# Aazmp/vp8oclenc

Measured on AMD Instinct MI355X. Metric: macroblocks/sec inter-frame (ME+DCT+loopfilter), 1080p, higher is better.
Workload: dtype u8/int32

## Files before the change

vp8oclenc_amd/csrc/kernels_s2.hip:

```cpp
#include <stdlib.h>
#include <string.h>

#include "vp8hip_dev.h"
#include "kernels_rc_dev.h"

namespace vp8 {

namespace {

constexpr uint32_t pk8(int a, int b, int c, int d) {
    return (uint32_t)(a & 255) | ((uint32_t)(b & 255) << 8) | ((uint32_t)(c & 255) << 16) | ((uint32_t)(d & 255) << 24);
}
constexpr int TAPS[5][6] = {{3, -16, 77, 77, -16, 3}, {1, -8, 36, 108, -11, 2}, {0, 0, 128, 0, 0, 0}, {2, -11, 108, 36, -8, 1}, {3, -16, 77, 77, -16, 3}};
struct OperandTable { uint32_t w[64][4]; };
constexpr OperandTable make_bh() {
    OperandTable t{};
    for (int l = 0; l < 64; ++l) {
        const int n = l & 31, xi = n >> 3, c = n & 7, xc = xi + (xi >> 1), s = xc >= 2 ? 1 : 0;
        for (int j = 0; j < 16; ++j) {
            const int k = 16 * (l >> 5) + j, tap = k - c - s;
            const int v = k == 31 ? 64 : (tap >= 0 && tap < 6) ? TAPS[xc][tap] : 0;
            t.w[l][j >> 2] |= (uint32_t)(v & 255) << (8 * (j & 3));
        }
    }
    return t;
}
constexpr OperandTable make_av() {
    OperandTable t{};
    for (int l = 0; l < 64; ++l) {
        const int m = l & 31, f = m >> 3, i = m & 7, yc = f + (f >> 1), s = yc >= 2 ? 1 : 0;
        for (int j = 0; j < 16; ++j) {
            const int k = 16 * (l >> 5) + j, tap = k - i - s;
            const int v = k == 31 ? 64 : (tap >= 0 && tap < 6) ? TAPS[yc][tap] : 0;
            t.w[l][j >> 2] |= (uint32_t)(v & 255) << (8 * (j & 3));
        }
    }
    return t;
}
static __device__ __constant__ const OperandTable K_BH = make_bh();
static __device__ __constant__ const OperandTable K_AV = make_av();

constexpr int HT_XC = 36;
constexpr int V_STRIDE = 20;
constexpr int WIN_ROW = 8;
__device__ __forceinline__ void lds_fence() { asm volatile("s_waitcnt lgkmcnt(0)" ::: "memory"); }

struct S2Args {
    Plane cur;
    Plane ref[3];
    const int16_t *net_in[3];
    int16_t *net_out[3];
    int32_t *bdiff[3];
    int refmap[3];
    int nrefs;
    int w, h, nblk, bw;
    uint32_t bw_inv;
    unsigned long long *clk;
};

__device__ __forceinline__ uint32_t umin(uint32_t a, uint32_t b) { return a < b ? a : b; }
template <int CTRL, int ROW_MASK = 0xf>
__device__ __forceinline__ uint32_t dpp(uint32_t v) {
    return (uint32_t)__builtin_amdgcn_update_dpp((int)v, (int)v, CTRL, ROW_MASK, 0xf, false);
}
template <int CTRL, int ROW_MASK = 0xf>
__device__ __forceinline__ uint32_t dpp_or_max(uint32_t v) {
    return (uint32_t)__builtin_amdgcn_update_dpp(-1, (int)v, CTRL, ROW_MASK, 0xf, false);
}
__device__ __forceinline__ uint32_t halfwave_min_upper(uint32_t key) {
    key = umin(key, dpp_or_max<0xb1>(key));
    key = umin(key, dpp_or_max<0x4e>(key));
    key = umin(key, dpp_or_max<0x141>(key));
    key = umin(key, dpp_or_max<0x140>(key));
    return umin(key, dpp_or_max<0x142, 0xa>(key));
}

typedef unsigned short us2 __attribute__((ext_vector_type(2)));
__device__ __forceinline__ unsigned short ashr7_pk_i8(int a, int b) { return __builtin_amdgcn_ashr_pk_i8_i32(a, b, 7); }
__device__ __forceinline__ uint32_t pack4(unsigned short lo, unsigned short hi) {
    const us2 v = {lo, hi};
    return __builtin_bit_cast(uint32_t, v);
}
__device__ __forceinline__ uint32_t round_pack4(const v16i &acc, int q) {
    return pack4(ashr7_pk_i8(acc[4 * q], acc[4 * q + 1]), ashr7_pk_i8(acc[4 * q + 2], acc[4 * q + 3]));
}
__device__ __forceinline__ v4i one_at_k31(v4i d, int upper) {
    d.w = (int)(((uint32_t)d.w & (0xffffffffu >> (8 & upper))) | (0x01000000u & (uint32_t)upper));
    return d;
}
__device__ __forceinline__ v16i mfma_round(v4i a, v4i b) {
    const v16i c = {0, 0, 0, 0, 0, 0, 0, 0, 0, 0, 0, 0, 0, 0, 0, 0};
    return __builtin_amdgcn_mfma_i32_32x32x32_i8(a, b, c, 0, 0, 0);
}

template <bool SPREAD>
__device__ __forceinline__ void search2_body(const S2Args &a, int wg_x, int ref_idx, int tn) {
    if (ref_idx >= a.nrefs) return;
    __shared__ __attribute__((aligned(16))) uint32_t s_HT[8][5 * HT_XC];
    __shared__ __attribute__((aligned(16))) uint32_t s_cz[8][32];
    __shared__ __attribute__((aligned(16))) uint32_t s_V[8][25 * V_STRIDE];
    uint32_t(*s_win)[25 * V_STRIDE] = s_V;
    int(*s_pre)[5 * HT_XC] = reinterpret_cast<int(*)[5 * HT_XC]>(s_HT);
    const int r = a.refmap[ref_idx];
    const int g = threadIdx.x >> 5, lane = threadIdx.x & 31;
    const int b = imin(wg_x * 8 + g, a.nblk - 1);
    const bool live = wg_x * 8 + g < a.nblk;
    const int by = a.bw == 1 ? b : (int)__umulhi((uint32_t)b, a.bw_inv), bx = b - by * a.bw;
    const int cx = bx * 8, cy = by * 8;
    const uint32_t nv = reinterpret_cast<const uint32_t *>(a.net_in[r])[b];
    const int nx = (int16_t)(nv & 0xffffu), ny = (int16_t)(nv >> 16);
    const int v0x = (int16_t)(nx * 4), v0y = (int16_t)(ny * 4);
    const int Lx = iclamp(cx + nx, 3 - EXT, a.w + EXT - 11), Ly = iclamp(cy + ny, 3 - EXT, a.h + EXT - 11);
    const Plane rf = a.ref[r];
    const int wl = threadIdx.x & 63, kh = wl >> 5, gp = g & ~1;
    const int g_n = tn >> 5, lane_n = tn & 31, wl_n = tn & 63, kh_n = wl_n >> 5, gp_n = g_n & ~1;
    {
        const int row = lane_n >> 1, half = lane_n & 1;
        v4i v;
        __builtin_memcpy(&v, rf.p + (ptrdiff_t)(Ly - 3 + row) * rf.stride + (Lx - 3) + 16 * half, 16);
        *reinterpret_cast<v4i *>(&s_win[g_n][row * WIN_ROW + 4 * half]) = v ^ (int)0x80808080u;
    }
    {
        const int sel = lane_n >> 4, row = (lane_n >> 1) & 7, half = lane_n & 1;
        const uint8_t *base = sel ? rf.p : a.cur.p;
        const int stride = sel ? rf.stride : a.cur.stride;
        const uint32_t v = *reinterpret_cast<const uint32_t *>(base + (ptrdiff_t)(cy + row) * stride + cx + 4 * half) ^ 0x80808080u;
        uint8_t *cz = reinterpret_cast<uint8_t *>(s_cz[g_n]) + sel * 64 + half * 32 + row;
#pragma unroll
        for (int j = 0; j < 4; ++j) cz[j * 8] = (uint8_t)(v >> (8 * j));
    }
    lds_fence();

    {
        const int m = wl & 31, m_n = wl_n & 31;
        const v4i aw = *reinterpret_cast<const v4i *>(&s_win[gp_n + (m_n >> 4)][(m_n & 15) * WIN_ROW + 4 * kh_n]);
        const v4i bh = *reinterpret_cast<const v4i *>(K_BH.w[wl_n]);
        const v16i acc = mfma_round(one_at_k31(aw, -kh_n), bh);
        const int xi = m >> 3, c = m & 7, xc = xi + (xi >> 1);
        uint32_t *ht = &s_HT[gp][xc * HT_XC + c * 4 + kh];
#pragma unroll
        for (int q = 0; q < 4; ++q) ht[(q >> 1) * (5 * HT_XC) + 2 * (q & 1)] = round_pack4(acc, q);
    }
    {
        const int c = lane_n & 7, rg = lane_n >> 3;
        const uint8_t *wb = reinterpret_cast<const uint8_t *>(s_win[g_n]) + 3 + c + rg * (16 * WIN_ROW);
        uint32_t v = 0;
#pragma unroll
        for (int rr = 0; rr < 4; ++rr) v |= (uint32_t)wb[rr * (4 * WIN_ROW)] << (8 * rr);
        s_HT[g_n][2 * HT_XC + c * 4 + rg] = v;
    }
    lds_fence();

    {
        const v4i av = *reinterpret_cast<const v4i *>(K_AV.w[wl_n]);
#pragma unroll
        for (int t = 0; t < 3; ++t) {
            const int ng = 32 * t + (wl & 31);
            const bool on = t < 2 || (wl & 31) < 16;
            const int blk = ng >= 40 ? 1 : 0, rem = on ? ng - 40 * blk : 0, xc = rem >> 3, c = rem & 7;
            const v4i hv = *reinterpret_cast<const v4i *>(&s_HT[gp + blk][xc * HT_XC + c * 4]);
            const v16i acc = mfma_round(av, one_at_k31(hv, -kh_n));
            if (on) {
                uint32_t *sv = &s_V[gp + blk][xc * V_STRIDE + c * 2 + kh];
#pragma unroll
                for (int f = 0; f < 4; ++f) sv[(f + (f >> 1)) * 5 * V_STRIDE] = round_pack4(acc, f);
                sv[2 * 5 * V_STRIDE] = kh ? __builtin_amdgcn_alignbyte((uint32_t)hv[2], (uint32_t)hv[1], 3)
                                          : __builtin_amdgcn_alignbyte((uint32_t)hv[1], (uint32_t)hv[0], 3);
            }
        }
    }
    lds_fence();
    {
        const int q = lane_n & 15, m = q >> 3, n = (q >> 2) & 1, j = q & 3;
        const uint32_t ccol = s_cz[g_n][(4 * n + j) * 2 + m];
        int *pre = &s_pre[g_n][q * 4 + (lane_n >> 4) * 2];
        pre[0] = dot4s(ccol, lane_n < 16 ? K_W_R0 : K_W_X, 0);
        pre[1] = dot4s(ccol, lane_n < 16 ? K_W_R2 : K_W_Y, 0);
    }
    lds_fence();

    const int k = lane;
    const int dx = k % 5 - 2, dy = k / 5 - 2;
    int qx = (int16_t)(cx * 4 + v0x + dx), qy = (int16_t)(cy * 4 + v0y + dy);
    if (k == 25) { qx = cx * 4; qy = cy * 4; }
    const bool valid = live && k < 26 && qx >= 0 && qx <= a.w * 4 - 32 && qy >= 0 && qy <= a.h * 4 - 32;
    int diff = 0;
    const v4i wa = metric_a(wl_n);
    auto cols4 = [](const uint32_t *src) { return v4i{(int)src[0], (int)src[2], (int)src[4], (int)src[6]}; };
    if (SPREAD) {
        int *q3 = &s_pre[g][64];
        const bool helper = lane >= 26;
        const uint32_t *own = k < 25 ? &s_V[g][k * V_STRIDE] : &s_cz[g][16];
        const uint32_t *hsrc = &s_V[g][(lane - 26) * 3 * V_STRIDE + 9];
        int *hdst = &q3[(lane - 26) * 3];
        auto metric = [&](const uint32_t *src, const int *pre16) { return weight_mfma(wa, load_pre16(pre16), cols4(src)); };
#pragma unroll
        for (int j = 0; j < 3; ++j) {
            const int c = metric(helper ? hsrc + j * V_STRIDE : own + (8 * (j & 1) + (j >> 1)), &s_pre[g][helper ? 48 : 16 * j]);
            *(helper ? hdst + j : &q3[31]) = c;
            diff += helper ? 0 : c;
        }
        __syncthreads();
        if ((int)(threadIdx.x >> 6) == (wg_x & 3)) {
            const int slot = wl >> 3, cand = 18 + (wl & 7);
            s_pre[slot][64 + cand] = metric((cand < 25 ? &s_V[slot][cand * V_STRIDE] : &s_cz[slot][16]) + 9, &s_pre[slot][48]);
        }
        __syncthreads();
        diff += q3[k < 26 ? k : 31];
    } else {
    const uint32_t *src = k < 25 ? &s_V[g][k * V_STRIDE] : &s_cz[g][16];
#pragma unroll
    for (int m = 0; m < 2; ++m)
#pragma unroll
        for (int n = 0; n < 2; ++n) diff += weight_mfma(wa, load_pre16(&s_pre[g][(m * 2 + n) * 16]), cols4(src + 8 * n + m));
    }
    if (k < 25) diff += (iabs(dx) + iabs(dy)) * 32;
    uint32_t key = (valid && diff < 0x7fff) ? ((uint32_t)diff << 8) | (uint32_t)k : 0xffffffffu;
    key = halfwave_min_upper(key);
    if (lane == 16 && live) {
        int bqx = (int16_t)(a.w * 4 - 32), bqy = (int16_t)(a.h * 4 - 32), md = 0x7fff;
        if (key != 0xffffffffu) {
            const int kk = key & 0xff;
            md = (int)(key >> 8);
            bqx = kk == 25 ? cx * 4 : (int16_t)(cx * 4 + v0x + (kk % 5 - 2));
            bqy = kk == 25 ? cy * 4 : (int16_t)(cy * 4 + v0y + (kk / 5 - 2));
        }
        const int vx = (int16_t)(bqx - cx * 4), vy = (int16_t)(bqy - cy * 4);
        if ((vx != 0) | (vy != 0)) md -= (iabs(vx - v0x) + iabs(vy - v0y)) * 32;
        reinterpret_cast<uint32_t *>(a.net_out[r])[b] = (uint32_t)(uint16_t)vx | ((uint32_t)(uint16_t)vy << 16);
        a.bdiff[r][b] = md;
    }
}

template <bool SPREAD, int ITER>
__device__ __forceinline__ void search2_groups(const S2Args &a, int grp, int ref_idx) {
    if (ITER == 1) { search2_body<SPREAD>(a, grp, ref_idx, (int)threadIdx.x); return; }
#pragma unroll 1
    for (int it = 0; it < ITER; ++it) {
        int tn = (int)threadIdx.x;
        asm volatile("" : "+v"(tn));
        search2_body<SPREAD>(a, grp * ITER + it, ref_idx, tn);
    }
}
template <bool SPREAD, int ITER>
__global__ __launch_bounds__(256, 4) void k_search2(S2Args a) {
    launch_clock_begin(a.clk);
    search2_groups<SPREAD, ITER>(a, xcd_band(blockIdx.x, gridDim.x), blockIdx.y);
    launch_clock_end(a.clk);
}
static_assert(sizeof(BatchOf<S2Args>) <= 4096, "a batch's argument blocks travel in the 4 KiB kernel-argument segment");
template <bool SPREAD, int ITER>
__global__ __launch_bounds__(256, 4) void k_search2_b(BatchOf<S2Args> b) {
    launch_clock_begin(b.item[0].clk);
    search2_groups<SPREAD, ITER>(b.item[blockIdx.z], xcd_band(blockIdx.x, gridDim.x), blockIdx.y);
    launch_clock_end(b.item[0].clk);
}
struct S2Scans { rc::ScanCore item[MAX_BATCH]; uint32_t mask; int nbx, wgs; };
static_assert(sizeof(BatchOf<S2Args>) + sizeof(S2Scans) <= 4096, "the kernel-argument segment");
template <bool SPREAD, int ITER>
__global__ __attribute__((amdgpu_waves_per_eu(7, 8))) __launch_bounds__(256) void k_search2_bs(BatchOf<S2Args> b, S2Scans sc) {
    if ((int)blockIdx.x >= sc.nbx) {
        const int wg = (int)blockIdx.x - sc.nbx;
        if (blockIdx.y == 0 && ((sc.mask >> blockIdx.z) & 1) && wg < sc.wgs) rc::strength_segments_body(b.item[blockIdx.z].cur, sc.item[blockIdx.z], wg, sc.wgs);
        return;
    }
    launch_clock_begin(b.item[0].clk);
    search2_groups<SPREAD, ITER>(b.item[blockIdx.z], xcd_band(blockIdx.x, sc.nbx), blockIdx.y);
    launch_clock_end(b.item[0].clk);
}
__global__ __launch_bounds__(256, 4) void k_search2_p(BatchOf<S2Args> b, int nbx, int maxrefs, int total) {
    for (int w = blockIdx.x; w < total; w += gridDim.x) {
        const int item = w / (nbx * maxrefs), rem = w - item * (nbx * maxrefs);
        const int ref_idx = rem / nbx, wg_x = rem - ref_idx * nbx;
        search2_body<false>(b.item[item], wg_x, ref_idx, (int)threadIdx.x);
        lds_fence();
    }
}

}

static S2Args search2_args(const Frame &cur, const RefSet &refs, const NetSet &nets, unsigned long long *clk) {
    S2Args a;
    a.clk = clk;
    a.cur = cur.Y[0];
    int n = 0;
    for (int r = 0; r < 3; ++r) {
        a.ref[r] = refs.ref[r].Y[0];
        a.net_in[r] = nets.net[r][1];
        a.net_out[r] = nets.net[r][0];
        a.bdiff[r] = nets.bdiff[r];
        if (refs.use[r]) a.refmap[n++] = r;
    }
    a.nrefs = n;
    for (int i = n; i < 3; ++i) a.refmap[i] = 0;
    a.w = a.cur.w;
    a.h = a.cur.h;
    a.bw = a.w / 8;
    a.bw_inv = (uint32_t)(((1ull << 32) + a.bw - 1) / a.bw);
    a.nblk = a.w * a.h / 64;
    return a;
}
static bool search2_spread() {
    static const bool on = [] { const char *v = getenv("VP8HIP_S2_SPREAD"); return !(v && v[0] == '0'); }();
    return on;
}
static int search2_iter(bool batch) {
    static const int forced = [] { const char *v = getenv("VP8HIP_S2_ITER"); const int k = v && v[0] ? atoi(v) : 0; return k == 1 || k == 2 || k == 4 ? k : 0; }();
    return forced ? forced : (batch ? 4 : 1);
}
static bool search2_skip() {
    static const bool skip = experiment_skip("s2");
    return skip;
}

void launch_search2(hipStream_t s, const Frame &cur, const RefSet &refs, const NetSet &nets, unsigned long long *clk) {
    const S2Args a = search2_args(cur, refs, nets, clk);
    if (a.nrefs == 0 || search2_skip()) return;
    const int nbx = (a.nblk + 7) / 8;
    if (!search2_spread()) VP8_LAUNCH((k_search2<false, 1>), dim3(nbx, a.nrefs), dim3(256), 0, s, a);
    else if (search2_iter(false) == 4) VP8_LAUNCH((k_search2<true, 4>), dim3((nbx + 3) / 4, a.nrefs), dim3(256), 0, s, a);
    else if (search2_iter(false) == 2) VP8_LAUNCH((k_search2<true, 2>), dim3((nbx + 1) / 2, a.nrefs), dim3(256), 0, s, a);
    else VP8_LAUNCH((k_search2<true, 1>), dim3(nbx, a.nrefs), dim3(256), 0, s, a);
}

bool launch_search2_batch(hipStream_t s, const Frame *const *cur, const RefSet *refs, const NetSet *const *nets, int n, unsigned long long *clk,
                          const ScanRequest *const *scan) {
    BatchOf<S2Args> b;
    b.n = n;
    int maxrefs = 0;
    for (int i = 0; i < n; ++i) {
        b.item[i] = search2_args(*cur[i], refs[i], *nets[i], clk);
        maxrefs = b.item[i].nrefs > maxrefs ? b.item[i].nrefs : maxrefs;
    }
    if (maxrefs == 0 || search2_skip()) return false;
    const int nbx = (b.item[0].nblk + 7) / 8;
    const int persist = persistent_workgroups();
    if (persist > 0 && nbx * maxrefs * n > persist) {
        VP8_LAUNCH(k_search2_p, dim3(persist), dim3(256), 0, s, b, nbx, maxrefs, nbx * maxrefs * n);
        return false;
    }
    S2Scans sc;
    sc.mask = 0;
    for (int i = 0; scan && i < n; ++i) {
        if (!scan[i]) continue;
        const ScanRequest &q = *scan[i];
        const Plane &y = b.item[i].cur;
        sc.mask |= 1u << i;
        sc.item[i] = rc::ScanCore{q.partial, q.partial + 2 * rc::MAX_PARTIALS, q.stats, q.sd, q.strength_out,
                                  rc::SegArgs{y.w * y.h, (y.h - 1) * (y.w - 1), q.is_key, q.refqi[0], q.refqi[1], q.refqi[2], q.refqi[3], q.qi_min}};
    }
    const int iter = search2_spread() ? search2_iter(true) : 1, ngrp = (nbx + iter - 1) / iter;
    if (!sc.mask) {
        if (!search2_spread()) VP8_LAUNCH((k_search2_b<false, 1>), dim3(nbx, maxrefs, n), dim3(256), 0, s, b);
        else if (iter == 4) VP8_LAUNCH((k_search2_b<true, 4>), dim3(ngrp, maxrefs, n), dim3(256), 0, s, b);
        else if (iter == 2) VP8_LAUNCH((k_search2_b<true, 2>), dim3(ngrp, maxrefs, n), dim3(256), 0, s, b);
        else VP8_LAUNCH((k_search2_b<true, 1>), dim3(nbx, maxrefs, n), dim3(256), 0, s, b);
        return false;
    }
    sc.nbx = ngrp;
    sc.wgs = (b.item[0].h + rc::ROWS_PER_BLOCK - 1) / rc::ROWS_PER_BLOCK;
    if (!search2_spread()) VP8_LAUNCH((k_search2_bs<false, 1>), dim3(nbx + sc.wgs, maxrefs, n), dim3(256), 0, s, b, sc);
    else if (iter == 4) VP8_LAUNCH((k_search2_bs<true, 4>), dim3(ngrp + sc.wgs, maxrefs, n), dim3(256), 0, s, b, sc);
    else if (iter == 2) VP8_LAUNCH((k_search2_bs<true, 2>), dim3(ngrp + sc.wgs, maxrefs, n), dim3(256), 0, s, b, sc);
    else VP8_LAUNCH((k_search2_bs<true, 1>), dim3(nbx + sc.wgs, maxrefs, n), dim3(256), 0, s, b, sc);
    return true;
}

}
```

Baseline: 69.19 million.

## Loop over all references inside one search2 workgroup and relayout subpel buffer

Batched search2 kernels now process every reference frame inside a single workgroup instead of one grid row per reference. The current-block precompute (dot products against the metric weights) is done once and reused across references. The interpolated-candidate LDS buffer is relaid so each candidate's four columns are contiguous and can be read with one vector load. The zero-MV reference block is stored into the same buffer. Default ITER for batches drops from 4 to 2 and the non-batch kernel switches to a waves_per_eu occupancy hint. This trades fewer workgroups and less parallelism for less redundant current-block work and fewer launches, with larger LDS per group.

```diff
diff --git a/vp8oclenc_amd/csrc/kernels_s2.hip b/vp8oclenc_amd/csrc/kernels_s2.hip
--- a/vp8oclenc_amd/csrc/kernels_s2.hip
+++ b/vp8oclenc_amd/csrc/kernels_s2.hip
@@ -41,7 +41,11 @@
 static __device__ __constant__ const OperandTable K_AV = make_av();
 
 constexpr int HT_XC = 36;
-constexpr int V_STRIDE = 20;
+constexpr int V_CAND = 4;
+constexpr int V_ROW = 26 * V_CAND;
+constexpr int V_SLOT = 4 * V_ROW;
+constexpr int V_ZERO = 25;
+constexpr int PRE_SLOT = 96;
 constexpr int WIN_ROW = 8;
 __device__ __forceinline__ void lds_fence() { asm volatile("s_waitcnt lgkmcnt(0)" ::: "memory"); }
 
@@ -93,166 +97,184 @@
     return __builtin_amdgcn_mfma_i32_32x32x32_i8(a, b, c, 0, 0, 0);
 }
 
-template <bool SPREAD>
+template <bool SPREAD, bool ALLREFS>
 __device__ __forceinline__ void search2_body(const S2Args &a, int wg_x, int ref_idx, int tn) {
-    if (ref_idx >= a.nrefs) return;
+    if (ALLREFS ? a.nrefs == 0 : ref_idx >= a.nrefs) return;
     __shared__ __attribute__((aligned(16))) uint32_t s_HT[8][5 * HT_XC];
-    __shared__ __attribute__((aligned(16))) uint32_t s_cz[8][32];
-    __shared__ __attribute__((aligned(16))) uint32_t s_V[8][25 * V_STRIDE];
-    uint32_t(*s_win)[25 * V_STRIDE] = s_V;
-    int(*s_pre)[5 * HT_XC] = reinterpret_cast<int(*)[5 * HT_XC]>(s_HT);
-    const int r = a.refmap[ref_idx];
+    __shared__ __attribute__((aligned(16))) uint32_t s_V[8][V_SLOT];
+    uint32_t(*s_win)[V_SLOT] = s_V;
+    __shared__ __attribute__((aligned(16))) int s_pre[8][PRE_SLOT];
+    int(*s_q3)[5 * HT_XC] = reinterpret_cast<int(*)[5 * HT_XC]>(s_HT);
     const int g = threadIdx.x >> 5, lane = threadIdx.x & 31;
+    const int wl = threadIdx.x & 63, kh = wl >> 5, gp = g & ~1;
     const int b = imin(wg_x * 8 + g, a.nblk - 1);
     const bool live = wg_x * 8 + g < a.nblk;
     const int by = a.bw == 1 ? b : (int)__umulhi((uint32_t)b, a.bw_inv), bx = b - by * a.bw;
     const int cx = bx * 8, cy = by * 8;
-    const uint32_t nv = reinterpret_cast<const uint32_t *>(a.net_in[r])[b];
-    const int nx = (int16_t)(nv & 0xffffu), ny = (int16_t)(nv >> 16);
-    const int v0x = (int16_t)(nx * 4), v0y = (int16_t)(ny * 4);
-    const int Lx = iclamp(cx + nx, 3 - EXT, a.w + EXT - 11), Ly = iclamp(cy + ny, 3 - EXT, a.h + EXT - 11);
-    const Plane rf = a.ref[r];
-    const int wl = threadIdx.x & 63, kh = wl >> 5, gp = g & ~1;
-    const int g_n = tn >> 5, lane_n = tn & 31, wl_n = tn & 63, kh_n = wl_n >> 5, gp_n = g_n & ~1;
     {
-        const int row = lane_n >> 1, half = lane_n & 1;
-        v4i v;
-        __builtin_memcpy(&v, rf.p + (ptrdiff_t)(Ly - 3 + row) * rf.stride + (Lx - 3) + 16 * half, 16);
-        *reinterpret_cast<v4i *>(&s_win[g_n][row * WIN_ROW + 4 * half]) = v ^ (int)0x80808080u;
-    }
-    {
-        const int sel = lane_n >> 4, row = (lane_n >> 1) & 7, half = lane_n & 1;
-        const uint8_t *base = sel ? rf.p : a.cur.p;
-        const int stride = sel ? rf.stride : a.cur.stride;
-        const uint32_t v = *reinterpret_cast<const uint32_t *>(base + (ptrdiff_t)(cy + row) * stride + cx + 4 * half) ^ 0x80808080u;
-        uint8_t *cz = reinterpret_cast<uint8_t *>(s_cz[g_n]) + sel * 64 + half * 32 + row;
-#pragma unroll
-        for (int j = 0; j < 4; ++j) cz[j * 8] = (uint8_t)(v >> (8 * j));
-    }
-    lds_fence();
-
-    {
-        const int m = wl & 31, m_n = wl_n & 31;
-        const v4i aw = *reinterpret_cast<const v4i *>(&s_win[gp_n + (m_n >> 4)][(m_n & 15) * WIN_ROW + 4 * kh_n]);
-        const v4i bh = *reinterpret_cast<const v4i *>(K_BH.w[wl_n]);
-        const v16i acc = mfma_round(one_at_k31(aw, -kh_n), bh);
-        const int xi = m >> 3, c = m & 7, xc = xi + (xi >> 1);
-        uint32_t *ht = &s_HT[gp][xc * HT_XC + c * 4 + kh];
-#pragma unroll
-        for (int q = 0; q < 4; ++q) ht[(q >> 1) * (5 * HT_XC) + 2 * (q & 1)] = round_pack4(acc, q);
-    }
-    {
-        const int c = lane_n & 7, rg = lane_n >> 3;
-        const uint8_t *wb = reinterpret_cast<const uint8_t *>(s_win[g_n]) + 3 + c + rg * (16 * WIN_ROW);
-        uint32_t v = 0;
-#pragma unroll
-        for (int rr = 0; rr < 4; ++rr) v |= (uint32_t)wb[rr * (4 * WIN_ROW)] << (8 * rr);
-        s_HT[g_n][2 * HT_XC + c * 4 + rg] = v;
-    }
-    lds_fence();
-
-    {
-        const v4i av = *reinterpret_cast<const v4i *>(K_AV.w[wl_n]);
-#pragma unroll
-        for (int t = 0; t < 3; ++t) {
-            const int ng = 32 * t + (wl & 31);
-            const bool on = t < 2 || (wl & 31) < 16;
-            const int blk = ng >= 40 ? 1 : 0, rem = on ? ng - 40 * blk : 0, xc = rem >> 3, c = rem & 7;
-            const v4i hv = *reinterpret_cast<const v4i *>(&s_HT[gp + blk][xc * HT_XC + c * 4]);
-            const v16i acc = mfma_round(av, one_at_k31(hv, -kh_n));
-            if (on) {
-                uint32_t *sv = &s_V[gp + blk][xc * V_STRIDE + c * 2 + kh];
-#pragma unroll
-                for (int f = 0; f < 4; ++f) sv[(f + (f >> 1)) * 5 * V_STRIDE] = round_pack4(acc, f);
-                sv[2 * 5 * V_STRIDE] = kh ? __builtin_amdgcn_alignbyte((uint32_t)hv[2], (uint32_t)hv[1], 3)
-                                          : __builtin_amdgcn_alignbyte((uint32_t)hv[1], (uint32_t)hv[0], 3);
-            }
-        }
-    }
-    lds_fence();
-    {
+        const int g_n = tn >> 5, lane_n = tn & 31;
+        uint32_t *tmp = reinterpret_cast<uint32_t *>(&s_pre[g_n][80]);
+        if (lane_n < 16) {
+            const int row = lane_n >> 1, half = lane_n & 1;
+            const uint32_t v = *reinterpret_cast<const uint32_t *>(a.cur.p + (ptrdiff_t)(cy + row) * a.cur.stride + cx + 4 * half) ^ 0x80808080u;
+            uint8_t *cz = reinterpret_cast<uint8_t *>(tmp) + half * 32 + row;
+#pragma unroll
+            for (int j = 0; j < 4; ++j) cz[j * 8] = (uint8_t)(v >> (8 * j));
+        }
+        lds_fence();
         const int q = lane_n & 15, m = q >> 3, n = (q >> 2) & 1, j = q & 3;
-        const uint32_t ccol = s_cz[g_n][(4 * n + j) * 2 + m];
+        const uint32_t ccol = tmp[(4 * n + j) * 2 + m];
         int *pre = &s_pre[g_n][q * 4 + (lane_n >> 4) * 2];
-        pre[0] = dot4s(ccol, lane_n < 16 ? K_W_R0 : K_W_X, 0);
-        pre[1] = dot4s(ccol, lane_n < 16 ? K_W_R2 : K_W_Y, 0);
-    }
-    lds_fence();
-
+        const int p0 = dot4s(ccol, lane_n < 16 ? K_W_R0 : K_W_X, 0), p1 = dot4s(ccol, lane_n < 16 ? K_W_R2 : K_W_Y, 0);
+        pre[0] = p0;
+        pre[1] = p1;
+        if (q >= 12) { pre[16] = p0; pre[17] = p1; pre[32] = p0; pre[33] = p1; }
+    }
     const int k = lane;
     const int dx = k % 5 - 2, dy = k / 5 - 2;
-    int qx = (int16_t)(cx * 4 + v0x + dx), qy = (int16_t)(cy * 4 + v0y + dy);
-    if (k == 25) { qx = cx * 4; qy = cy * 4; }
-    const bool valid = live && k < 26 && qx >= 0 && qx <= a.w * 4 - 32 && qy >= 0 && qy <= a.h * 4 - 32;
-    int diff = 0;
-    const v4i wa = metric_a(wl_n);
-    auto cols4 = [](const uint32_t *src) { return v4i{(int)src[0], (int)src[2], (int)src[4], (int)src[6]}; };
-    if (SPREAD) {
-        int *q3 = &s_pre[g][64];
-        const bool helper = lane >= 26;
-        const uint32_t *own = k < 25 ? &s_V[g][k * V_STRIDE] : &s_cz[g][16];
-        const uint32_t *hsrc = &s_V[g][(lane - 26) * 3 * V_STRIDE + 9];
-        int *hdst = &q3[(lane - 26) * 3];
-        auto metric = [&](const uint32_t *src, const int *pre16) { return weight_mfma(wa, load_pre16(pre16), cols4(src)); };
-#pragma unroll
-        for (int j = 0; j < 3; ++j) {
-            const int c = metric(helper ? hsrc + j * V_STRIDE : own + (8 * (j & 1) + (j >> 1)), &s_pre[g][helper ? 48 : 16 * j]);
-            *(helper ? hdst + j : &q3[31]) = c;
-            diff += helper ? 0 : c;
-        }
-        __syncthreads();
-        if ((int)(threadIdx.x >> 6) == (wg_x & 3)) {
-            const int slot = wl >> 3, cand = 18 + (wl & 7);
-            s_pre[slot][64 + cand] = metric((cand < 25 ? &s_V[slot][cand * V_STRIDE] : &s_cz[slot][16]) + 9, &s_pre[slot][48]);
-        }
-        __syncthreads();
-        diff += q3[k < 26 ? k : 31];
+    const uint32_t kcode = k < 25 ? (uint32_t)((iabs(dx) + iabs(dy)) * 32 * 256 + (dy + 2) * 8 + dx + 2) : 40u;
+    const v4i wa = metric_a(wl);
+
+    auto one_reference = [&](int ri) {
+        int tr = tn;
+        if (ALLREFS) asm volatile("" : "+v"(tr));
+        const int g_n = tr >> 5, lane_n = tr & 31, wl_n = tr & 63, kh_n = wl_n >> 5, gp_n = g_n & ~1;
+        const int r = a.refmap[ri];
+        const uint32_t nv = reinterpret_cast<const uint32_t *>(a.net_in[r])[b];
+        const int nx = (int16_t)(nv & 0xffffu), ny = (int16_t)(nv >> 16);
+        const int v0x = (int16_t)(nx * 4), v0y = (int16_t)(ny * 4);
+        const int Lx = iclamp(cx + nx, 3 - EXT, a.w + EXT - 11), Ly = iclamp(cy + ny, 3 - EXT, a.h + EXT - 11);
+        const Plane rf = a.ref[r];
+        {
+            const int row = lane_n >> 1, half = lane_n & 1;
+            v4i v;
+            __builtin_memcpy(&v, rf.p + (ptrdiff_t)(Ly - 3 + row) * rf.stride + (Lx - 3) + 16 * half, 16);
+            *reinterpret_cast<v4i *>(&s_win[g_n][row * WIN_ROW + 4 * half]) = v ^ (int)0x80808080u;
+        }
+        const uint32_t zv = *reinterpret_cast<const uint32_t *>(rf.p + (ptrdiff_t)(cy + ((lane_n >> 1) & 7)) * rf.stride + cx + 4 * (lane_n & 1)) ^ 0x80808080u;
+        lds_fence();
+
+        {
+            const int m = wl & 31, m_n = wl_n & 31;
+            const v4i aw = *reinterpret_cast<const v4i *>(&s_win[gp_n + (m_n >> 4)][(m_n & 15) * WIN_ROW + 4 * kh_n]);
+            const v4i bh = *reinterpret_cast<const v4i *>(K_BH.w[wl_n]);
+            const v16i acc = mfma_round(one_at_k31(aw, -kh_n), bh);
+            const int xi = m >> 3, c = m & 7, xc = xi + (xi >> 1);
+            uint32_t *ht = &s_HT[gp][xc * HT_XC + c * 4 + kh];
+#pragma unroll
+            for (int q = 0; q < 4; ++q) ht[(q >> 1) * (5 * HT_XC) + 2 * (q & 1)] = round_pack4(acc, q);
+        }
+        {
+            const int c = lane_n & 7, rg = lane_n >> 3;
+            const uint8_t *wb = reinterpret_cast<const uint8_t *>(s_win[g_n]) + 3 + c + rg * (16 * WIN_ROW);
+            uint32_t v = 0;
+#pragma unroll
+            for (int rr = 0; rr < 4; ++rr) v |= (uint32_t)wb[rr * (4 * WIN_ROW)] << (8 * rr);
+            s_HT[g_n][2 * HT_XC + c * 4 + rg] = v;
+        }
+        {
+            const int row = (lane_n >> 1) & 7, half = lane_n & 1;
+            uint8_t *z = reinterpret_cast<uint8_t *>(&s_V[g_n][((row >> 2) * 2 + half) * V_ROW + V_ZERO * V_CAND]) + (row & 3);
+#pragma unroll
+            for (int j = 0; j < 4; ++j) z[j * 4] = (uint8_t)(zv >> (8 * j));
+        }
+        lds_fence();
+
+        {
+            const v4i av = *reinterpret_cast<const v4i *>(K_AV.w[wl_n]);
+#pragma unroll
+            for (int t = 0; t < 3; ++t) {
+                const int ng = 32 * t + (wl & 31);
+                const bool on = t < 2 || (wl & 31) < 16;
+                const int blk = ng >= 40 ? 1 : 0, rem = on ? ng - 40 * blk : 0, xc = rem >> 3, c = rem & 7;
+                const v4i hv = *reinterpret_cast<const v4i *>(&s_HT[gp + blk][xc * HT_XC + c * 4]);
+                const v16i acc = mfma_round(av, one_at_k31(hv, -kh_n));
+                if (on) {
+                    uint32_t *sv = &s_V[gp + blk][(kh * 2 + (c >> 2)) * V_ROW + xc * V_CAND + (c & 3)];
+#pragma unroll
+                    for (int f = 0; f < 4; ++f) sv[(f + (f >> 1)) * 5 * V_CAND] = round_pack4(acc, f);
+                    sv[2 * 5 * V_CAND] = kh ? __builtin_amdgcn_alignbyte((uint32_t)hv[2], (uint32_t)hv[1], 3)
+                                            : __builtin_amdgcn_alignbyte((uint32_t)hv[1], (uint32_t)hv[0], 3);
+                }
+            }
+        }
+        lds_fence();
+
+        int qx = (int16_t)(cx * 4 + v0x + dx), qy = (int16_t)(cy * 4 + v0y + dy);
+        if (k == 25) { qx = cx * 4; qy = cy * 4; }
+        const bool valid = live && k < 26 && qx >= 0 && qx <= a.w * 4 - 32 && qy >= 0 && qy <= a.h * 4 - 32;
+        int diff = 0;
+        auto metric = [&](const uint32_t *src, const int *pre16) { return weight_mfma(wa, load_pre16(pre16), *reinterpret_cast<const v4i *>(src)); };
+        if (SPREAD) {
+            int *q3 = &s_q3[g][64];
+            const bool helper = lane >= 26;
+            const uint32_t *src = helper ? &s_V[g][3 * V_ROW + (lane - 26) * 3 * V_CAND] : &s_V[g][k * V_CAND];
+            const int step = helper ? V_CAND : V_ROW;
+            const int *pre = &s_pre[g][helper ? 48 : 0];
+            int *dst = &q3[helper ? (lane - 26) * 3 : 29];
+#pragma unroll
+            for (int j = 0; j < 3; ++j) {
+                const int c = metric(src + j * step, pre + 16 * j);
+                dst[j] = c;
+                diff += c;
+            }
+            __syncthreads();
+            if ((int)(threadIdx.x >> 6) == (wg_x & 3)) {
+                const int slot = wl >> 3, cand = 18 + (wl & 7);
+                s_q3[slot][64 + cand] = metric(&s_V[slot][3 * V_ROW + cand * V_CAND], &s_pre[slot][48]);
+            }
+            __syncthreads();
+            diff += q3[k < 26 ? k : 31];
+        } else {
+            const uint32_t *src = &s_V[g][imin(k, V_ZERO) * V_CAND];
+#pragma unroll
+            for (int bb = 0; bb < 4; ++bb) diff += metric(src + bb * V_ROW, &s_pre[g][bb * 16]);
+        }
+        uint32_t key = ((uint32_t)diff << 8) + kcode;
+        key = (valid && key < (0x7fffu << 8)) ? key : 0xffffffffu;
+        key = halfwave_min_upper(key);
+        if (lane == 16 && live) {
+            int vx = (int16_t)((int16_t)(a.w * 4 - 32) - cx * 4), vy = (int16_t)((int16_t)(a.h * 4 - 32) - cy * 4), md = 0x7fff;
+            if (key != 0xffffffffu) {
+                const int kk = key & 0xff;
+                md = (int)(key >> 8);
+                vx = kk == 40 ? 0 : (int16_t)(v0x + (kk & 7) - 2);
+                vy = kk == 40 ? 0 : (int16_t)(v0y + (kk >> 3) - 2);
+            }
+            if ((vx != 0) | (vy != 0)) md -= (iabs(vx - v0x) + iabs(vy - v0y)) * 32;
+            reinterpret_cast<uint32_t *>(a.net_out[r])[b] = (uint32_t)(uint16_t)vx | ((uint32_t)(uint16_t)vy << 16);
+            a.bdiff[r][b] = md;
+        }
+    };
+    if (ALLREFS) {
+#pragma unroll 1
+        for (int ri = 0; ri < a.nrefs; ++ri) one_reference(ri);
     } else {
-    const uint32_t *src = k < 25 ? &s_V[g][k * V_STRIDE] : &s_cz[g][16];
-#pragma unroll
-    for (int m = 0; m < 2; ++m)
-#pragma unroll
-        for (int n = 0; n < 2; ++n) diff += weight_mfma(wa, load_pre16(&s_pre[g][(m * 2 + n) * 16]), cols4(src + 8 * n + m));
-    }
-    if (k < 25) diff += (iabs(dx) + iabs(dy)) * 32;
-    uint32_t key = (valid && diff < 0x7fff) ? ((uint32_t)diff << 8) | (uint32_t)k : 0xffffffffu;
-    key = halfwave_min_upper(key);
-    if (lane == 16 && live) {
-        int bqx = (int16_t)(a.w * 4 - 32), bqy = (int16_t)(a.h * 4 - 32), md = 0x7fff;
-        if (key != 0xffffffffu) {
-            const int kk = key & 0xff;
-            md = (int)(key >> 8);
-            bqx = kk == 25 ? cx * 4 : (int16_t)(cx * 4 + v0x + (kk % 5 - 2));
-            bqy = kk == 25 ? cy * 4 : (int16_t)(cy * 4 + v0y + (kk / 5 - 2));
-        }
-        const int vx = (int16_t)(bqx - cx * 4), vy = (int16_t)(bqy - cy * 4);
-        if ((vx != 0) | (vy != 0)) md -= (iabs(vx - v0x) + iabs(vy - v0y)) * 32;
-        reinterpret_cast<uint32_t *>(a.net_out[r])[b] = (uint32_t)(uint16_t)vx | ((uint32_t)(uint16_t)vy << 16);
-        a.bdiff[r][b] = md;
-    }
-}
-
-template <bool SPREAD, int ITER>
+        one_reference(ref_idx);
+    }
+}
+
+template <bool SPREAD, int ITER, bool ALLREFS>
 __device__ __forceinline__ void search2_groups(const S2Args &a, int grp, int ref_idx) {
-    if (ITER == 1) { search2_body<SPREAD>(a, grp, ref_idx, (int)threadIdx.x); return; }
+    if (ITER == 1 && !ALLREFS) { search2_body<SPREAD, ALLREFS>(a, grp, ref_idx, (int)threadIdx.x); return; }
 #pragma unroll 1
     for (int it = 0; it < ITER; ++it) {
         int tn = (int)threadIdx.x;
         asm volatile("" : "+v"(tn));
-        search2_body<SPREAD>(a, grp * ITER + it, ref_idx, tn);
+        search2_body<SPREAD, ALLREFS>(a, grp * ITER + it, ref_idx, tn);
     }
 }
 template <bool SPREAD, int ITER>
-__global__ __launch_bounds__(256, 4) void k_search2(S2Args a) {
+__global__ __attribute__((amdgpu_waves_per_eu(7, 8))) __launch_bounds__(256) void k_search2(S2Args a) {
     launch_clock_begin(a.clk);
-    search2_groups<SPREAD, ITER>(a, xcd_band(blockIdx.x, gridDim.x), blockIdx.y);
+    search2_groups<SPREAD, ITER, false>(a, xcd_band(blockIdx.x, gridDim.x), blockIdx.y);
     launch_clock_end(a.clk);
 }
 static_assert(sizeof(BatchOf<S2Args>) <= 4096, "a batch's argument blocks travel in the 4 KiB kernel-argument segment");
 template <bool SPREAD, int ITER>
-__global__ __launch_bounds__(256, 4) void k_search2_b(BatchOf<S2Args> b) {
+__global__ __attribute__((amdgpu_waves_per_eu(7, 8))) __launch_bounds__(256) void k_search2_b(BatchOf<S2Args> b) {
     launch_clock_begin(b.item[0].clk);
-    search2_groups<SPREAD, ITER>(b.item[blockIdx.z], xcd_band(blockIdx.x, gridDim.x), blockIdx.y);
+    search2_groups<SPREAD, ITER, true>(b.item[blockIdx.z], xcd_band(blockIdx.x, gridDim.x), 0);
     launch_clock_end(b.item[0].clk);
 }
 struct S2Scans { rc::ScanCore item[MAX_BATCH]; uint32_t mask; int nbx, wgs; };
@@ -261,18 +283,18 @@
 __global__ __attribute__((amdgpu_waves_per_eu(7, 8))) __launch_bounds__(256) void k_search2_bs(BatchOf<S2Args> b, S2Scans sc) {
     if ((int)blockIdx.x >= sc.nbx) {
         const int wg = (int)blockIdx.x - sc.nbx;
-        if (blockIdx.y == 0 && ((sc.mask >> blockIdx.z) & 1) && wg < sc.wgs) rc::strength_segments_body(b.item[blockIdx.z].cur, sc.item[blockIdx.z], wg, sc.wgs);
+        if (((sc.mask >> blockIdx.z) & 1) && wg < sc.wgs) rc::strength_segments_body(b.item[blockIdx.z].cur, sc.item[blockIdx.z], wg, sc.wgs);
         return;
     }
     launch_clock_begin(b.item[0].clk);
-    search2_groups<SPREAD, ITER>(b.item[blockIdx.z], xcd_band(blockIdx.x, sc.nbx), blockIdx.y);
+    search2_groups<SPREAD, ITER, true>(b.item[blockIdx.z], xcd_band(blockIdx.x, sc.nbx), 0);
     launch_clock_end(b.item[0].clk);
 }
 __global__ __launch_bounds__(256, 4) void k_search2_p(BatchOf<S2Args> b, int nbx, int maxrefs, int total) {
     for (int w = blockIdx.x; w < total; w += gridDim.x) {
         const int item = w / (nbx * maxrefs), rem = w - item * (nbx * maxrefs);
         const int ref_idx = rem / nbx, wg_x = rem - ref_idx * nbx;
-        search2_body<false>(b.item[item], wg_x, ref_idx, (int)threadIdx.x);
+        search2_body<false, false>(b.item[item], wg_x, ref_idx, (int)threadIdx.x);
         lds_fence();
     }
 }
@@ -305,8 +327,8 @@
     return on;
 }
 static int search2_iter(bool batch) {
-    static const int forced = [] { const char *v = getenv("VP8HIP_S2_ITER"); const int k = v && v[0] ? atoi(v) : 0; return k == 1 || k == 2 || k == 4 ? k : 0; }();
-    return forced ? forced : (batch ? 4 : 1);
+    static const int forced = [] { const char *v = getenv("VP8HIP_S2_ITER"); const int k = v && v[0] ? atoi(v) : 0; return k == 1 || k == 2 ? k : 0; }();
+    return forced ? forced : (batch ? 2 : 1);
 }
 static bool search2_skip() {
     static const bool skip = experiment_skip("s2");
@@ -318,7 +340,6 @@
     if (a.nrefs == 0 || search2_skip()) return;
     const int nbx = (a.nblk + 7) / 8;
     if (!search2_spread()) VP8_LAUNCH((k_search2<false, 1>), dim3(nbx, a.nrefs), dim3(256), 0, s, a);
-    else if (search2_iter(false) == 4) VP8_LAUNCH((k_search2<true, 4>), dim3((nbx + 3) / 4, a.nrefs), dim3(256), 0, s, a);
     else if (search2_iter(false) == 2) VP8_LAUNCH((k_search2<true, 2>), dim3((nbx + 1) / 2, a.nrefs), dim3(256), 0, s, a);
     else VP8_LAUNCH((k_search2<true, 1>), dim3(nbx, a.nrefs), dim3(256), 0, s, a);
 }
@@ -351,18 +372,16 @@
     }
     const int iter = search2_spread() ? search2_iter(true) : 1, ngrp = (nbx + iter - 1) / iter;
     if (!sc.mask) {
-        if (!search2_spread()) VP8_LAUNCH((k_search2_b<false, 1>), dim3(nbx, maxrefs, n), dim3(256), 0, s, b);
-        else if (iter == 4) VP8_LAUNCH((k_search2_b<true, 4>), dim3(ngrp, maxrefs, n), dim3(256), 0, s, b);
-        else if (iter == 2) VP8_LAUNCH((k_search2_b<true, 2>), dim3(ngrp, maxrefs, n), dim3(256), 0, s, b);
-        else VP8_LAUNCH((k_search2_b<true, 1>), dim3(nbx, maxrefs, n), dim3(256), 0, s, b);
+        if (!search2_spread()) VP8_LAUNCH((k_search2_b<false, 1>), dim3(nbx, 1, n), dim3(256), 0, s, b);
+        else if (iter == 2) VP8_LAUNCH((k_search2_b<true, 2>), dim3(ngrp, 1, n), dim3(256), 0, s, b);
+        else VP8_LAUNCH((k_search2_b<true, 1>), dim3(nbx, 1, n), dim3(256), 0, s, b);
         return false;
     }
     sc.nbx = ngrp;
     sc.wgs = (b.item[0].h + rc::ROWS_PER_BLOCK - 1) / rc::ROWS_PER_BLOCK;
-    if (!search2_spread()) VP8_LAUNCH((k_search2_bs<false, 1>), dim3(nbx + sc.wgs, maxrefs, n), dim3(256), 0, s, b, sc);
-    else if (iter == 4) VP8_LAUNCH((k_search2_bs<true, 4>), dim3(ngrp + sc.wgs, maxrefs, n), dim3(256), 0, s, b, sc);
-    else if (iter == 2) VP8_LAUNCH((k_search2_bs<true, 2>), dim3(ngrp + sc.wgs, maxrefs, n), dim3(256), 0, s, b, sc);
-    else VP8_LAUNCH((k_search2_bs<true, 1>), dim3(nbx + sc.wgs, maxrefs, n), dim3(256), 0, s, b, sc);
+    if (!search2_spread()) VP8_LAUNCH((k_search2_bs<false, 1>), dim3(nbx + sc.wgs, 1, n), dim3(256), 0, s, b, sc);
+    else if (iter == 2) VP8_LAUNCH((k_search2_bs<true, 2>), dim3(ngrp + sc.wgs, 1, n), dim3(256), 0, s, b, sc);
+    else VP8_LAUNCH((k_search2_bs<true, 1>), dim3(nbx + sc.wgs, 1, n), dim3(256), 0, s, b, sc);
     return true;
 }
 
```

Measured after the change: 70.52 million (median of 6 runs). 1.02x the previous value.
